# YulioTech/Yulio-Raytracer

Hardware: AMD Instinct MI355X
Metric: Mrays/s (Sponza stand-in 2048^2 64spp, closest+shadow queries) (higher is better)
Workload: dtype f32

## Files before the change

yulio-raytracer_amd/csrc/kernels/k_firsthit.h:

```cpp
#pragma once

#include "yrt_camera.h"
#include "yrt_shade.h"
#include "yrt_surface.h"
#include "yrt_traverse.h"

namespace yrt {

__global__ __launch_bounds__(64) void k_debug(SceneView sv, FrameView fv, int maxDepth, int spp,
                                             float* __restrict__ fbFloat, uint8_t* __restrict__ fbRGB8,
                                             int rgb8Stride) {
  const GpuRenderParams& rp = *fv.rp;
  const GpuCamera& cam = *fv.cam;
  const int tile = blockIdx.x * blockDim.x + threadIdx.x;
  if (tile >= rp.numTilesX * rp.numTilesY) return;
  DevRandom rnd;
  rnd.setSeed(tile * 1024);
  const int x0 = (tile % rp.numTilesX) * 16, y0 = (tile / rp.numTilesX) * 16;
  for (int dy = 0; dy < 16; dy++) {
    const int iy = y0 + dy;
    const float fy = iy * rp.rcpHeight;
    if (iy >= rp.height) continue;
    for (int dx = 0; dx < 16; dx++) {
      const int ix = x0 + dx;
      const float fx = ix * rp.rcpWidth;
      if (ix >= rp.width) continue;
      for (int i = 0; i < spp; i++) {
        V3 org, dir;
        camera_ray(cam, fx, fy, org, dir);
        float tnear = 0.f, tfar = __int_as_float(0x7f800000);
        Hit h;
        h.tri = -1;
        int id0 = -1, id1 = -1;
        for (int depth = 0; depth < maxDepth; depth++) {
          h = closest_hit(sv.qnodes, sv.tris, org, dir, tnear, tfar);
          if (h.tri < 0) {
            id0 = id1 = -1;
            break;
          }
          const int g = sv.triGeom[h.tri];
          id0 = g;
          id1 = h.tri - sv.geoms[g].triBase;
          if (depth + 1 < maxDepth) {
            const int4 idx = sv.indices[h.tri];
            const V3 p0 = ld3(sv.positions[idx.x]), p1 = ld3(sv.positions[idx.y]), p2 = ld3(sv.positions[idx.z]);
            V3 e1, e2;
            yrt_tri_edges(&p0.x, &p1.x, &p2.x, &e1.x, &e2.x);
            V3 Nf = normalize(cross(e1, e2));
            if (dot(-dir, Nf) < 0) Nf = -Nf;
            const float u1 = rnd.getFloat();
            const float u2 = rnd.getFloat();
            float pdf;
            const V3 norg = org + 0.999f * h.t * dir;
            dir = cosine_hemi(u1, u2, Nf, pdf);
            org = norg;
            tnear = 4.0f * kUlp;
            tfar = __int_as_float(0x7f800000);
          }
        }
        V3 c;
        if (id0 < 0) c = v3s(1.0f);
        else
          c = v3(((3434553u * ((unsigned)(id0 + id1 + 3243))) % 255) / 255.0f,
                 ((7342453u * ((unsigned)(id0 + id1 + 8237))) % 255) / 255.0f,
                 ((9234454u * ((unsigned)(id0 + id1 + 2343))) % 255) / 255.0f);
        if (fbFloat) {
          float* o = fbFloat + ((size_t)iy * rp.width + ix) * 3;
          o[0] = c.x;
          o[1] = c.y;
          o[2] = c.z;
        }
        if (fbRGB8) {
          uint8_t* o = fbRGB8 + (size_t)iy * rgb8Stride + 3 * ix;
          o[0] = (uint8_t)clampf(c.x * 255.0f, 0.0f, 255.0f);
          o[1] = (uint8_t)clampf(c.y * 255.0f, 0.0f, 255.0f);
          o[2] = (uint8_t)clampf(c.z * 255.0f, 0.0f, 255.0f);
        }
      }
    }
  }
}

__global__ __launch_bounds__(YRT_TRACE_BLOCK) void k_pick(SceneView sv, const GpuCamera* camp, float x, float y,
                                                          float4* out) {
  if (threadIdx.x != 0) return;
  V3 org, dir;
  camera_ray(*camp, x, y, org, dir);
  const Hit h = closest_hit(sv.qnodes, sv.tris, org, dir, 0.f, __int_as_float(0x7f800000));
  const V3 p = org + h.t * dir;
  out[0] = make_float4(p.x, p.y, p.z, __int_as_float(h.tri));
}

template <bool ALBEDO>
__global__ __launch_bounds__(YRT_TRACE_BLOCK) void k_guides(SceneView sv, const GpuCamera* camp, int width, int height,
                                                            float4* __restrict__ pos4, float4* __restrict__ nrm4,
                                                            float4* __restrict__ albedo4) {
  const long long i = (long long)blockIdx.x * blockDim.x + threadIdx.x;
  if (i >= (long long)width * height) return;
  const int y = (int)(i / width), x = (int)(i - (long long)y * width);
  V3 org, dir;
  camera_ray(*camp, (float(x) + 0.5f) / float(width), (float(y) + 0.5f) / float(height), org, dir);
  const Hit h = closest_hit(sv.qnodes, sv.tris, org, dir, 0.f, __int_as_float(0x7f800000));
  if (h.tri < 0) {
    pos4[i] = make_float4(0.f, 0.f, 0.f, __int_as_float(0x7f800000));
    nrm4[i] = make_float4(0.f, 0.f, 0.f, 0.f);
    if constexpr (ALBEDO) albedo4[i] = make_float4(0.f, 0.f, 0.f, 0.f);
    return;
  }
  DG dg;
  const float4* tsr = (const float4*)(sv.triShade + h.tri);
  const float4 r0 = tsr[0];
  const int g = __float_as_int(r0.w);
  post_intersect(sv, sv.geoms[g], tsr, r0, org, dir, h.t, h.u, h.v, h.tri, dg, false, 0.f);
  V3 n = dg.Ns;
  if (dot(n, dir) > 0.f) n = -n;
  pos4[i] = make_float4(dg.P.x, dg.P.y, dg.P.z, h.t);
  nrm4[i] = make_float4(n.x, n.y, n.z, 1.f);
  if constexpr (ALBEDO) {
    V3 a = v3s(0.f);
    if (dg.light < 0 && dg.material >= 0) {
      DG sdg = dg;
      if (dot(sdg.Ng, dir) > 0.f) {
        sdg.Ng = -sdg.Ng;
        sdg.Ns = -sdg.Ns;
      }
      BRDFSet bs;
      const GpuGeomRec& gr = sv.geomRecs[g];
      shade_material<YRT_ALL_MATS>(sv, gr.m, gr.t0, sdg.material, 0, sdg, bs);
#pragma unroll
      for (int k = 0; k < YRT_MAX_COMPS; ++k)
        if (k < bs.n && comp_type(bs.c[k].kind) == BT_DIFFUSE_REFLECTION) a = a + bs.c[k].R;
    }
    if (a == v3s(0.f)) a = v3s(1.f);
    albedo4[i] = make_float4(a.x, a.y, a.z, 1.f);
  }
}

}
```

yulio-raytracer_amd/csrc/kernels/k_shade.h:

```cpp
#pragma once

#include "yrt_camera.h"
#include "yrt_surface.h"

namespace yrt {

#ifndef YRT_SHADE_WAVES
#define YRT_SHADE_WAVES 4
#endif
#ifndef YRT_SHADE_WAVES_ALL
#define YRT_SHADE_WAVES_ALL 2
#endif
#ifndef YRT_SHADE_WAVES_MP
#define YRT_SHADE_WAVES_MP YRT_SHADE_WAVES
#endif
#ifdef YRT_PATH_DEBUG
__device__ int g_dbgPath[2] = {-1, -1};
__device__ float g_dbgTrace[32 * 32];
#endif

template <unsigned MM>
__global__ __launch_bounds__(YRT_BLOCK) __attribute__((amdgpu_waves_per_eu(
    MM == (YRT_ALL_MATS | YRT_ALL_LIGHTS) ? YRT_SHADE_WAVES_ALL
    : (MM & mat_bit(MAT_METALLIC_PAINT)) ? YRT_SHADE_WAVES_MP
                                         : YRT_SHADE_WAVES))) void k_shade(SceneView sv, FrameView fv, PathBuffers pb, BatchInfo bi,
                                                   int depthLevel) {
#ifdef YRT_SHADE_PROF
  unsigned long long sprof[8] = {0, 0, 0, 0, 0, 0, 0, 0};
  unsigned long long tprev = __builtin_amdgcn_s_memtime();
#define SPROF_AT(k)                                            \
  do {                                                         \
    const unsigned long long t_ = __builtin_amdgcn_s_memtime(); \
    sprof[k] += t_ - tprev;                                    \
    tprev = t_;                                                \
  } while (0)
#endif
#if defined(YRT_SHADE_PROF) && YRT_SHADE_PROF == 1
#define SPROF_MARK(k) SPROF_AT(k)
#else
#define SPROF_MARK(k) ((void)0)
#endif
#if defined(YRT_SHADE_PROF) && YRT_SHADE_PROF == 2
#define SPROF_FINE(k) SPROF_AT(k)
#else
#define SPROF_FINE(k) ((void)0)
#endif
  const YRT_CONST GpuRenderParams& rp = const_ref(fv.rp);
  __shared__ QMap qm;
  __shared__ float sstash[7 * YRT_MAX_COMPS * YRT_BLOCK];
  qmap_load(qm, pb.counters + qcounter_index(depthLevel, 0, 0), YRT_QSEGS);
  const int n = (int)qm.pre[YRT_QSEGS];
  const int cur = depthLevel & 1;
  const int numDirect = sv.numDirectLights;
  for (int base = blockIdx.x * blockDim.x; base < n; base += gridDim.x * blockDim.x) {
    const unsigned ql = (unsigned)base + threadIdx.x;
    const bool active = (int)ql < n;
    const int q = active ? qmap_phys(qm, pb.segCap, ql) : 0;
    const int oseg = qseg_of((unsigned)base + (threadIdx.x & ~63u));
    unsigned* nextCount = pb.counters + qcounter_index(depthLevel + 1, 0, oseg);
    unsigned* shadowCount = pb.counters + qcounter_index(depthLevel, 1, oseg);
    int path = 0;
    V3 org = v3s(0.f), dir = v3s(0.f), thr = v3s(0.f), L = v3s(0.f);
    int meta = 0, depth = 0, rec = 0, pixelId = 0, s = 0, medium = 0;
    bool ignoreVL = false, unbent = false, isHit = false, useDirect = false;
    bool haveL = false;
    float4 h = make_float4(0.f, 0.f, 0.f, 0.f);
    DG dg;
    BRDFSet bs;
    bs.n = 0;
#pragma unroll
    for (int k = 0; k < YRT_MAX_COMPS; ++k) {
      bs.c[k].kind = 0;
      bs.c[k].R = v3s(0.f);
      bs.c[k].a = bs.c[k].b = bs.c[k].c = 0.f;
    }
    V3 wo = v3s(0.f);
    int px = 0, py = 0;
    SPROF_MARK(7);
    SPROF_FINE(7);
    if (active) {
      path = pb.qPath[cur][q];
      h = pb.hit[q];
      if (depthLevel == 0) {
        thr = v3s(1.f);
        meta = 1 << 9;
        L = v3s(0.f);
        haveL = true;
      } else {
        const float4 t4 = pb.qThr[cur][q];
        thr = v3(t4.x, t4.y, t4.z);
        meta = __float_as_int(t4.w);
      }
      depth = meta & 255;
      ignoreVL = (meta >> 8) & 1;
      unbent = (meta >> 9) & 1;
      medium = (meta >> 10) & 0xFFFF;
      s = fastdiv(path, bi.divPixels);
      const int i = path - s * bi.numPixels;
      batch_pixel(rp, bi, i, px, py);
      pixelId = py * rp.width + px;
      isHit = __float_as_int(h.w) >= 0;
    }
    if (active && (isHit || sv.numEnvDir > 0)) {
      const float4 d = pb.qDir[cur][q];
      dir = v3(d.x, d.y, d.z);
      wo = -dir;
    }
    SPROF_MARK(0);
    if (active && !isHit) {
      {
        const int x = px, y = py;
        if (fv.backplateTexels && unbent) {
          rec = fv.pixelSets[pixelId] * rp.spp + s;
          const float fx = (float(x) + samp(fv, 0, rec)) * rp.rcpWidth;
          const float fy = (float(y) + samp(fv, 1, rec)) * rp.rcpHeight;
          const GpuImage& bp = fv.backplate;
          const int bx = max(0, min((int)(fx * (float)bp.width), bp.width - 1));
          const int by = max(0, min((int)(fy * (float)bp.height), bp.height - 1));
          float c[4];
          texel(bp, fv.backplateTexels, bx, by, c);
          if (!haveL) { const float4 l4 = pb.pathL[path]; L = v3(l4.x, l4.y, l4.z); haveL = true; }
          L = L + thr * v3(c[0], c[1], c[2]);
        } else if (!ignoreVL) {
          for (int j = 0; j < sv.numEnvLights; ++j) {
            if (!haveL) { const float4 l4 = pb.pathL[path]; L = v3(l4.x, l4.y, l4.z); haveL = true; }
            L = L + thr * env_Le<lights_of<MM>()>(sv, const_ref(sv.lights + const_ref(sv.envLights + j)), wo);
          }
          if (sv.numEnvZero > 0 && !(fabsf(thr.x) <= 3.40282347e38f && fabsf(thr.y) <= 3.40282347e38f && fabsf(thr.z) <= 3.40282347e38f)) {
            if (!haveL) { const float4 l4 = pb.pathL[path]; L = v3(l4.x, l4.y, l4.z); haveL = true; }
            L = L + thr * v3s(0.f);
          }
        }
      }
    }
    SPROF_MARK(1);
    bool backfacing = false;
    int g = 0;
    if (active && isHit) {
      const int gid = __float_as_int(h.w);
      const float4* tsr = (const float4*)(sv.triShade + gid);
      const float4 r0 = tsr[0];
      const float4 o = pb.qOrg[cur][q];
      org = v3(o.x, o.y, o.z);
      rec = fv.pixelSets[pixelId] * rp.spp + s;
      g = __float_as_int(r0.w);
      const GpuGeomRec& gr = sv.geomRecs[g];
      const int mat = gr.g.material;
      const bool wantT = mat >= 0 && (((MM & mat_bit(MAT_OBJ)) && gr.m.type == MAT_OBJ && gr.m.tex[4] >= 0) ||
                                      ((MM & mat_bit(MAT_BRUSHED_METAL)) && gr.m.type == MAT_BRUSHED_METAL));
      post_intersect(sv, gr.g, tsr, r0, org, dir, h.x, h.y, h.z, gid, dg, wantT, pb.qTime[0] ? samp(fv, 4, rec) : 0.f);
      if (dot(dg.Ng, dir) > 0.f) {
        backfacing = true;
        dg.Ng = -dg.Ng;
        dg.Ns = -dg.Ns;
      }
    }
    SPROF_MARK(2);
    if (active && isHit) {
      if (dg.material >= 0) shade_material<MM>(sv, sv.geomRecs[g].m, sv.geomRecs[g].t0, dg.material, medium, dg, bs);
      if (!ignoreVL && dg.light >= 0 && !backfacing) {
        const GpuLight& al = sv.lights[dg.light];
        if (!haveL) { const float4 l4 = pb.pathL[path]; L = v3(l4.x, l4.y, l4.z); haveL = true; }
        L = L + thr * v3(al.L[0], al.L[1], al.L[2]);
      }
#pragma unroll
      for (int k = 0; k < YRT_MAX_COMPS; ++k)
        if (k < bs.n) useDirect |= (comp_type(bs.c[k].kind) & BT_DIFFUSE) != 0;
      dg_frame(dg);
    }
    SPROF_MARK(3);

    bool cont = false;
    V3 nwi = v3s(0.f), nthr = v3s(0.f);
    int nmeta = 0;
    bool doSample = false;
    float4 sd = make_float4(0.f, 0.f, 0.f, 0.f);
    float sy = 0.f, ss = 0.f;
    if (active && isHit) {
      bool stop = depth >= rp.maxDepth - 1;
      if (!stop && rp.rrDepth > 0 && depth >= rp.rrDepth - 1) {
        const float qrr = fminf(reduce_max(thr) * 1.f * 1.f, .95f);
        if (samp(fv, 5 + rp.firstScatterTypeSampleID + depth, rec) >= qrr) stop = true;
      }
      if (!stop) {
        const int d2 = rp.firstScatterSampleID + depth;
        sd = samp_dir(fv, d2, rec);
        if constexpr ((comps_of(MM) & kCompsRawSy) != 0u) sy = samp(fv, 5 + rp.dim1D + 2 * d2 + 1, rec);
        ss = samp(fv, 5 + rp.firstScatterTypeSampleID + depth, rec);
        doSample = true;
      }
    }
    SPROF_FINE(0);
    float spdf = 0.f;
    uint32_t stype = 0;
    V3 sc = v3s(0.f);
    if (doSample)
      sc = set_sample<comps_of(MM)>(bs, sv.materials, wo, dg, sd, sy, ss, nwi, spdf, stype, sstash + threadIdx.x);
    SPROF_FINE(1);
    if (doSample) {
      {
        V3 c = sc;
        const float pdf = spdf;
        const uint32_t type = stype;
        if (!(c == v3s(0.f) || pdf <= 0.f)) {
          if (MM & mat_bit(MAT_DIELECTRIC)) {
            const float4 T = sv.media[medium];
            if (!(T.x == 1.f && T.y == 1.f && T.z == 1.f)) c = c * v3(yrt_powf(T.x, h.x), yrt_powf(T.y, h.x), yrt_powf(T.z, h.x));
            if ((type & BT_TRANSMISSION) && dg.material >= 0) {
              const GpuMaterial& mt = sv.materials[dg.material];
              if (mt.type == MAT_DIELECTRIC) medium = medium == mt.media[1] ? mt.media[0] : mt.media[1];
            }
          }
          nthr = thr * c * rcpf_(pdf);
          const bool nIgnore = (type & BT_DIFFUSE) != 0;
          const bool nUnbent = unbent && (nwi == dir);
          if (!(reduce_max(nthr) < rp.minContribution)) {
            cont = true;
            nmeta = (depth + 1) | ((nIgnore ? 1 : 0) << 8) | ((nUnbent ? 1 : 0) << 9) | (medium << 10);
          }
        }
      }
    }
    SPROF_MARK(4);
    if (haveL) pb.pathL[path] = make_float4(L.x, L.y, L.z, 0.f);
    auto cont_store = [&](unsigned nq) {
      if (pb.qTime[0]) pb.qTime[cur ^ 1][nq] = samp(fv, 4, rec);
      pb.qPath[cur ^ 1][nq] = path;
      pb.qOrg[cur ^ 1][nq] = make_float4(dg.P.x, dg.P.y, dg.P.z, dg.error * rp.epsilon);
      pb.qDir[cur ^ 1][nq] = make_float4(nwi.x, nwi.y, nwi.z, __int_as_float(0x7f800000));
      pb.qThr[cur ^ 1][nq] = make_float4(nthr.x, nthr.y, nthr.z, __int_as_float(nmeta));
    };
    auto light_term = [&](int k, V3& wi, float& tfar, V3& contrib) -> bool {
      const int li = const_ref(sv.directLights + k);
      const YRT_CONST GpuLight& lt = const_ref(sv.lights + li);
      const bool lit = active && isHit && useDirect && (lt.illumMask & dg.illumMask) != 0;
      V3 Ls = v3s(0.f);
      float pdf = 0.f;
      if (lit) {
        if (lt.precomputed >= 0) {
          const float* ls = fv.lightSamples + ((size_t)rec * fv.numLightSlots + lt.precomputed) * 8;
          wi = v3(ls[0], ls[1], ls[2]);
          pdf = ls[3];
          Ls = v3(ls[4], ls[5], ls[6]);
        } else {
          float4 lsd = make_float4(0.f, 0.f, 0.f, 0.f);
          float lsx = 0.f, lsy = 0.f;
          if ((1u << lt.type) & kLightsDir) lsd = samp_dir(fv, rp.lightSampleID, rec);
          if ((lights_of<MM>() & kLightsRawS) != 0u && ((1u << lt.type) & kLightsRawS)) {
            lsx = samp(fv, 5 + rp.dim1D + 2 * rp.lightSampleID, rec);
            lsy = samp(fv, 5 + rp.dim1D + 2 * rp.lightSampleID + 1, rec);
          }
          Ls = light_sample<lights_of<MM>()>(lt, dg, lsd, lsx, lsy, wi, pdf);
        }
      }
      SPROF_FINE(3);
      const bool lsOk = lit && !(Ls == v3s(0.f) || pdf == 0.f);
      V3 brdf = v3s(0.f);
      if (lsOk) brdf = set_eval<comps_of(MM)>(bs, sv.materials, wo, dg, wi, BT_DIFFUSE);
      SPROF_FINE(4);
      if (lsOk && !(brdf == v3s(0.f))) {
        const float r01 = hash_u01(rp.frameSeed, (uint32_t)pixelId, (uint32_t)s, (uint32_t)(depth * 64 + li));
        const float shadowRayJitterLength = 2.f * rp.tMaxShadowRay * rp.tMaxShadowJitter * r01 -
                                            rp.tMaxShadowRay * rp.tMaxShadowJitter;
        float tMax = rp.tMaxShadowRay + shadowRayJitterLength;
        const float dotProduct = dot(wi, ld3(rp.up));
        if (dotProduct <= 0.f) tMax += rp.tMaxShadowRay * 100.f * smoothstepf(0.f, 1.f, fabsf(dotProduct));
        tfar = tMax - dg.error * rp.epsilon;
        contrib = thr * Ls * brdf * rcpf_(pdf);
        return true;
      }
      return false;
    };
    auto shadow_store = [&](unsigned si, const V3& wi, float tfar, const V3& contrib) {
      if (pb.sTime) pb.sTime[si] = samp(fv, 4, rec);
      pb.sOrg[si] = make_float4(dg.P.x, dg.P.y, dg.P.z, dg.error * rp.epsilon);
      pb.sDir[si] = make_float4(wi.x, wi.y, wi.z, tfar);
      pb.sContrib[si] = make_float4(contrib.x, contrib.y, contrib.z, __int_as_float(path));
    };
    {
      bool got;
      const unsigned nq = oseg * pb.segCap + wave_append(nextCount, cont, got);
      if (got) cont_store(nq);
      SPROF_MARK(5);
      SPROF_FINE(2);
      for (int k = 0; k < numDirect; ++k) {
        V3 wi = v3s(0.f), contrib = v3s(0.f);
        float tfar = 0.f;
        const bool pred = light_term(k, wi, tfar, contrib);
        SPROF_FINE(5);
        bool sgot;
        const unsigned si = oseg * pb.shSegCap + wave_append(shadowCount, pred, sgot);
        if (sgot) shadow_store(si, wi, tfar, contrib);
        if (active && !pb.fuseShadow) pb.shFirst[(size_t)q * numDirect + k] = sgot ? (int)si : -1;
        SPROF_FINE(6);
      }
    }
    SPROF_MARK(6);
#ifdef YRT_PATH_DEBUG
    if (active && pixelId == g_dbgPath[0] && s == g_dbgPath[1] && depth < 32) {
      float* o = g_dbgTrace + depth * 32;
      if (!haveL) { const float4 l4 = pb.pathL[path]; L = v3(l4.x, l4.y, l4.z); }
      const float r[32] = {1.f, isHit ? (float)__float_as_int(h.w) : -1.f, h.x, h.y, h.z, thr.x, thr.y, thr.z,
                           dg.P.x, dg.P.y, dg.P.z, dg.Ns.x, dg.Ns.y, dg.Ns.z, L.x, L.y, L.z, nwi.x, nwi.y, nwi.z,
                           spdf, sc.x, sc.y, sc.z, nthr.x, nthr.y, nthr.z, dir.x, dir.y, dir.z, org.x, (float)useDirect};
      for (int k = 0; k < 32; ++k) o[k] = r[k];
    }
#endif
  }
#ifdef YRT_SHADE_PROF
  if (threadIdx.x == 0)
    for (int k = 0; k < 8; ++k) atomicAdd(&g_traceProfile[k], sprof[k]);
#endif
}

__global__ __launch_bounds__(YRT_BLOCK) void k_shadow_resolve(PathBuffers pb, int depthLevel, int numLights) {
  __shared__ QMap qm;
  qmap_load(qm, pb.counters + qcounter_index(depthLevel, 0, 0), YRT_QSEGS);
  const int n = (int)qm.pre[YRT_QSEGS];
  const int cur = depthLevel & 1;
  for (int ql = blockIdx.x * blockDim.x + threadIdx.x; ql < n; ql += gridDim.x * blockDim.x) {
    const int q = qmap_phys(qm, pb.segCap, (unsigned)ql);
    bool any = false;
    for (int li = 0; li < numLights; ++li) any |= pb.shFirst[(size_t)q * numLights + li] >= 0;
    if (!any) continue;
    float4* Lp = &pb.pathL[pb.qPath[cur][q]];
    const float4 l4 = *Lp;
    V3 L = v3(l4.x, l4.y, l4.z);
    for (int li = 0; li < numLights; ++li) {
      const int si = pb.shFirst[(size_t)q * numLights + li];
      if (si < 0 || pb.sOcc[si]) continue;
      const float4 c = pb.sContrib[si];
      L = L + v3(c.x, c.y, c.z);
    }
    *Lp = make_float4(L.x, L.y, L.z, 0.f);
  }
}

__device__ int g_dbgPixel[3] = {-1, -1, 0};
__device__ float4* g_dbgOut = nullptr;

__global__ __launch_bounds__(YRT_BLOCK) void k_resolve_pixels(FrameView fv, PathBuffers pb, BatchInfo bi,
                                                            float* __restrict__ fbFloat, uint8_t* __restrict__ fbRGB8,
                                                            int rgb8Stride, float4* __restrict__ accu, int accumulate) {
  const YRT_CONST GpuRenderParams& rp = const_ref(fv.rp);
  const size_t frameStride = (size_t)rp.width * rp.height;
  for (int i = blockIdx.x * blockDim.x + threadIdx.x; i < bi.numPixels; i += gridDim.x * blockDim.x) {
    int x, y, f;
    if (!batch_pixel(rp, bi, i, x, y, f)) continue;
    V3 L = v3s(0.f);
    for (int s = 0; s < rp.spp; ++s) {
      const float4 l4 = pb.pathL[(size_t)s * bi.numPixels + i];
      L = L + v3(l4.x, l4.y, l4.z);
    }
    if (g_dbgPixel[0] == y * rp.width + x && g_dbgPixel[1] == f && g_dbgOut)
      for (int s = 0; s < min(rp.spp, g_dbgPixel[2]); ++s) g_dbgOut[s] = pb.pathL[(size_t)s * bi.numPixels + i];
    const size_t pix = (size_t)f * frameStride + (size_t)y * rp.width + x;
    float4 a = make_float4(L.x, L.y, L.z, (float)rp.spp);
    if (accumulate) {
      const float4 c = accu[pix];
      a = make_float4(c.x + L.x, c.y + L.y, c.z + L.z, c.w + (float)rp.spp);
    }
    accu[pix] = a;
    V3 L0 = accumulate ? v3(a.x, a.y, a.z) * rcpf_(a.w) : L * rcpf_((float)rp.spp);
    if (rp.gamma != 1.0f) L0 = v3(yrt_powf(L0.x, rp.rcpGamma), yrt_powf(L0.y, rp.rcpGamma), yrt_powf(L0.z, rp.rcpGamma));
    if (rp.vignetting) {
      const float rw = rcpf_(0.5f * float(rp.width));
      const float vx = (float(x) - 0.5f * float(rp.width)) * rw, vy = (float(y) - 0.5f * float(rp.height)) * rw;
      const float d = sqrtf(vx * vx + vy * vy);
      L0 = L0 * yrt_powf(yrt_cosf(d * 0.5f), 3.0f);
    }
    if (fbFloat) {
      float* o = fbFloat + pix * 3;
      o[0] = L0.x;
      o[1] = L0.y;
      o[2] = L0.z;
    }
    if (fbRGB8) {
      uint8_t* o = fbRGB8 + ((size_t)f * rp.height + y) * rgb8Stride + 3 * x;
      o[0] = (uint8_t)clampf(L0.x * 255.0f, 0.0f, 255.0f);
      o[1] = (uint8_t)clampf(L0.y * 255.0f, 0.0f, 255.0f);
      o[2] = (uint8_t)clampf(L0.z * 255.0f, 0.0f, 255.0f);
    }
  }
}

#undef SPROF_AT
#undef SPROF_MARK
#undef SPROF_FINE

}
```

yulio-raytracer_amd/csrc/kernels/yrt_surface.h:

```cpp
#pragma once

#include "yrt_shade.h"
#include "yrt_wave.h"
#include "../common/yrt_tri_record.h"

namespace yrt {


struct TriRecordSource {
  static constexpr bool kTangentArrays = false;
  const float4* __restrict__ rec;
  float4 r0;
  __device__ __forceinline__ void edges(V3& e1, V3& e2, V3& dPdu, V3& dPdv) const {
    const float4 r1 = rec[1];
    e1 = v3(r0.x, r0.y, r0.z); e2 = v3(r1.x, r1.y, r1.z);
    dPdu = -e1; dPdv = e2;
  }
  __device__ __forceinline__ void normals(V3& n0, V3& n1, V3& n2) const {
    const float4 r2 = rec[2], r3 = rec[3], r4 = rec[4];
    n0 = v3(r2.x, r2.y, r2.z); n1 = v3(r2.w, r3.x, r3.y); n2 = v3(r3.z, r3.w, r4.x);
  }
  __device__ __forceinline__ void texcoords(float2& st0, float2& st1, float2& st2) const {
    const float4 r4 = rec[4], r5 = rec[5];
    st0 = make_float2(r4.y, r4.z); st1 = make_float2(r4.w, r5.x); st2 = make_float2(r5.y, r5.z);
  }
};

struct TriIndexedSource {
  static constexpr bool kTangentArrays = true;
  const SceneView& sv;
  const int4 idx;
  const float time;
  const bool moving;
  __device__ __forceinline__ void edges(V3& e1, V3& e2, V3& dPdu, V3& dPdv) const {
    V3 p0 = ld3(sv.positions[idx.x]), p1 = ld3(sv.positions[idx.y]), p2 = ld3(sv.positions[idx.z]);
    if (moving) {
      p0 = p0 + time * ld3(sv.motions[idx.x]);
      p1 = p1 + time * ld3(sv.motions[idx.y]);
      p2 = p2 + time * ld3(sv.motions[idx.z]);
    }
    yrt_tri_edges(&p0.x, &p1.x, &p2.x, &e1.x, &e2.x);
    dPdu = p1 - p0; dPdv = p2 - p0;
  }
  __device__ __forceinline__ void normals(V3& n0, V3& n1, V3& n2) const {
    n0 = ld3(sv.normals[idx.x]); n1 = ld3(sv.normals[idx.y]); n2 = ld3(sv.normals[idx.z]);
  }
  __device__ __forceinline__ void texcoords(float2& st0, float2& st1, float2& st2) const {
    st0 = sv.texcoords[idx.x]; st1 = sv.texcoords[idx.y]; st2 = sv.texcoords[idx.z];
  }
  __device__ __forceinline__ V3 tangent(int k, float w, float u, float v) const {
    return w * ld3(sv.tangents[2 * idx.x + k]) + u * ld3(sv.tangents[2 * idx.y + k]) +
           v * ld3(sv.tangents[2 * idx.z + k]);
  }
};

__device__ __forceinline__ void post_intersect(const SceneView& sv, const GpuGeom& geom,
                                               const float4* __restrict__ rec, float4 r0, V3 org, V3 dir, float t,
                                               float u, float v, int gid, DG& dg, bool wantTangents, float time) {
  dg.material = geom.material;
  dg.light = geom.light;
  dg.illumMask = geom.illumMask;
  dg.shadowMask = geom.shadowMask;
  dg.P = org + t * dir;
  dg.s = u; dg.t = v;
  dg.Tx = dg.Ty = v3s(0.f);
  auto mesh = [&](const auto src) {
    V3 e1, e2, dPdu, dPdv;
    src.edges(e1, e2, dPdu, dPdv);
    const float w = 1.0f - u - v;
    dg.Ns = dg.Ng = normalize(cross(e1, e2));
    const bool meshNormals = geom.kind == GEOM_MESH_NORMALS;
    if (meshNormals || (geom.flags & GF_NORMALS)) {
      V3 n0, n1, n2;
      src.normals(n0, n1, n2);
      V3 Ns = w * n0 + u * n1 + v * n2;
      const float len2 = dot(Ns, Ns);
      Ns = len2 > 0 ? Ns * rsqrtf_(len2) : dg.Ng;
      if (dot(Ns, dg.Ng) < 0) Ns = -Ns;
      dg.Ns = Ns;
    }
    if (meshNormals) {
      dg.Tx = dPdu; dg.Ty = dPdv;
      return;
    }
    float dsdu = 1, dtdu = 0, dsdv = 0, dtdv = 1;
    if (geom.flags & GF_TEXCOORDS) {
      float2 st0, st1, st2;
      src.texcoords(st0, st1, st2);
      dg.s = st0.x * w + st1.x * u + st2.x * v;
      dg.t = st0.y * w + st1.y * u + st2.y * v;
      dsdu = st1.x - st0.x; dtdu = st1.y - st0.y;
      dsdv = st2.x - st0.x; dtdv = st2.y - st0.y;
    }
    if (!wantTangents) return;
    const V3 dPds = normalize(dPdu * dtdv - dPdv * dtdu);
    dg.Tx = normalize(dPds - dot(dPds, dg.Ns) * dg.Ns);
    const V3 dPdt = normalize(dPdv * dsdu - dPdu * dsdv);
    dg.Ty = normalize(dPdt - dot(dPdt, dg.Ns) * dg.Ns);
    if constexpr (src.kTangentArrays) {
      if (geom.flags & GF_TANGENT_X) dg.Tx = src.tangent(0, w, u, v);
      if (geom.flags & GF_TANGENT_Y) dg.Ty = src.tangent(1, w, u, v);
    }
  };
  if (geom.kind == GEOM_TRIANGLE)
    dg.Ns = dg.Ng = v3(geom.Ng[0], geom.Ng[1], geom.Ng[2]);
  else if (geom.flags & (GF_MOTION | GF_TANGENT_X | GF_TANGENT_Y))
    mesh(TriIndexedSource{sv, sv.indices[gid], time, (geom.flags & GF_MOTION) != 0});
  else
    mesh(TriRecordSource{rec, r0});
  dg.error = fmaxf(fabsf(t), reduce_max(absv(dg.P)));
}

__device__ __forceinline__ void add_comp(BRDFSet& bs, int kind, uint32_t type, V3 R, float a = 0.f, float b = 0.f,
                                         float c = 0.f) {
  (void)type;
#pragma unroll
  for (int i = 0; i < YRT_MAX_COMPS; ++i) {
    const bool w = i == bs.n;
    bs.c[i].kind = w ? kind : bs.c[i].kind;
    bs.c[i].R = v3(w ? R.x : bs.c[i].R.x, w ? R.y : bs.c[i].R.y, w ? R.z : bs.c[i].R.z);
    bs.c[i].a = w ? a : bs.c[i].a;
    bs.c[i].b = w ? b : bs.c[i].b;
    bs.c[i].c = w ? c : bs.c[i].c;
  }
  bs.n = bs.n < YRT_MAX_COMPS ? bs.n + 1 : bs.n;
}

template <unsigned MM>
__device__ __forceinline__ void shade_material(const SceneView& sv, const GpuMaterial& m, const GpuTexture& t0, int matId,
                                               int medium, DG& dg, BRDFSet& bs) {
  bs.n = 0;
  const float idBits = __int_as_float(matId);
  switch (m.type) {
    case MAT_PLASTIC:
      if constexpr (!(MM & mat_bit(MAT_PLASTIC))) break;
      add_comp(bs, C_DIEL_LAYER_LAMB, BT_DIFFUSE_REFLECTION, v3(m.p[0], m.p[1], m.p[2]), m.p[6], m.p[7]);
      if (m.p[4] == 0.0f) add_comp(bs, C_DIEL_REFL, BT_SPECULAR_REFLECTION, v3s(0.f), m.p[8], 1.0f);
      else add_comp(bs, C_MICROFACET, BT_GLOSSY_REFLECTION, v3s(1.f), 1.0f, m.p[3], m.p[5]);
      break;
    case MAT_DIELECTRIC:
      if constexpr (!(MM & mat_bit(MAT_DIELECTRIC))) break;
      if (medium == m.media[0]) {
        add_comp(bs, C_DIEL_REFL, BT_SPECULAR_REFLECTION, v3s(0.f), m.p[8], 1.0f);
        add_comp(bs, C_DIEL_TRANS, BT_SPECULAR_TRANSMISSION, v3s(0.f), m.p[8]);
      } else {
        add_comp(bs, C_DIEL_REFL, BT_SPECULAR_REFLECTION, v3s(0.f), m.p[9], 1.0f);
        add_comp(bs, C_DIEL_TRANS, BT_SPECULAR_TRANSMISSION, v3s(0.f), m.p[9]);
      }
      break;
    case MAT_MIRROR:
      if constexpr (!(MM & mat_bit(MAT_MIRROR))) break;
      add_comp(bs, C_REFLECTION, BT_SPECULAR_REFLECTION, v3(m.p[0], m.p[1], m.p[2]));
      break;
    case MAT_METAL:
      if constexpr (!(MM & mat_bit(MAT_METAL))) break;
      if (m.p[9] == 0.0f) add_comp(bs, C_CONDUCTOR, BT_SPECULAR_REFLECTION, v3(m.p[0], m.p[1], m.p[2]), 0.f, 0.f, idBits);
      else add_comp(bs, C_MICRO_COND, BT_GLOSSY_REFLECTION, v3(m.p[0], m.p[1], m.p[2]), m.p[10], 0.f, idBits);
      break;
    case MAT_BRUSHED_METAL:
      if constexpr (!(MM & mat_bit(MAT_BRUSHED_METAL))) break;
      if (m.p[9] == 0.0f || m.p[10] == 0.0f)
        add_comp(bs, C_CONDUCTOR, BT_SPECULAR_REFLECTION, v3(m.p[0], m.p[1], m.p[2]), 0.f, 0.f, idBits);
      else
        add_comp(bs, C_MICRO_ANISO, BT_GLOSSY_REFLECTION, v3(m.p[0], m.p[1], m.p[2]), m.p[11], m.p[12], idBits);
      break;
    case MAT_VELVET:
      if constexpr (!(MM & mat_bit(MAT_VELVET))) break;
      add_comp(bs, C_MINNAERT, BT_DIFFUSE_REFLECTION, v3(m.p[0], m.p[1], m.p[2]), m.p[3]);
      add_comp(bs, C_VELVETY, BT_DIFFUSE_REFLECTION, v3(m.p[4], m.p[5], m.p[6]), m.p[7]);
      break;
    case MAT_MATTE:
      if constexpr (!(MM & mat_bit(MAT_MATTE))) break;
      add_comp(bs, C_LAMBERT, BT_DIFFUSE_REFLECTION, v3(m.p[0], m.p[1], m.p[2]));
      break;
    case MAT_MATTE_TEXTURED:
      if constexpr (!(MM & mat_bit(MAT_MATTE_TEXTURED))) break;
      if (m.tex[0] >= 0) {
        float c[4];
        tex_get_rec(t0, sv.texels, sv.texQuads, m.p[2] * dg.s + m.p[0], m.p[3] * dg.t + m.p[1], c);
        add_comp(bs, C_LAMBERT, BT_DIFFUSE_REFLECTION, v3(c[0], c[1], c[2]));
      }
      break;
    case MAT_METALLIC_PAINT:
      if constexpr (!(MM & mat_bit(MAT_METALLIC_PAINT))) break;
      add_comp(bs, C_DIEL_REFL, BT_SPECULAR_REFLECTION, v3s(0.f), m.p[4], 1.0f);
      add_comp(bs, C_DIEL_LAYER_LAMB, BT_DIFFUSE_REFLECTION, v3(m.p[0], m.p[1], m.p[2]), m.p[5], m.p[6]);
      break;
    case MAT_METALLIC_GLITTER:
      if constexpr (!(MM & mat_bit(MAT_METALLIC_GLITTER))) break;
      add_comp(bs, C_DIEL_REFL, BT_SPECULAR_REFLECTION, v3s(0.f), m.p[4], 1.0f);
      add_comp(bs, C_DIEL_LAYER_LAMB, BT_DIFFUSE_REFLECTION, v3(m.p[0], m.p[1], m.p[2]), m.p[5], m.p[6]);
      add_comp(bs, C_DIEL_LAYER_GLITTER, BT_GLOSSY_REFLECTION, v3(m.p[7], m.p[8], m.p[9]), m.p[5], m.p[6], m.p[10]);
      break;
    case MAT_OBJ: {
      if constexpr (!(MM & mat_bit(MAT_OBJ))) break;
      float c[4];
      if (m.tex[4] >= 0) {
        tex_get(sv.textures, sv.images, sv.texels, sv.texQuads, m.tex[4], dg.s, dg.t, c);
        const V3 b = v3(2.0f * c[0] - 1.0f, 2.0f * c[1] - 1.0f, 2.0f * c[2] - 1.0f);
        dg.Ns = normalize(b.x * dg.Tx + b.y * dg.Ty + b.z * dg.Ns);
      }
      float d = m.p[0];
      if (m.tex[0] >= 0) {
        tex_get_rec(t0, sv.texels, sv.texQuads, dg.s, dg.t, c);
        d *= c[0];
      }
      if (d < 1.0f) add_comp(bs, C_TRANSMISSION, BT_SPECULAR_TRANSMISSION, v3s(1.0f - d));
      V3 Kd = d * v3(m.p[1], m.p[2], m.p[3]);
      if (m.tex[1] >= 0) {
        tex_get(sv.textures, sv.images, sv.texels, sv.texQuads, m.tex[1], dg.s, dg.t, c);
        Kd = Kd * v3(c[0], c[1], c[2]);
      }
      if (Kd != v3s(0.f)) add_comp(bs, C_LAMBERT, BT_DIFFUSE_REFLECTION, Kd);
      float Ns = m.p[7];
      if (m.tex[3] >= 0) {
        tex_get(sv.textures, sv.images, sv.texels, sv.texQuads, m.tex[3], dg.s, dg.t, c);
        Ns *= c[0];
      }
      V3 Ks = d * v3(m.p[4], m.p[5], m.p[6]);
      if (m.tex[2] >= 0) {
        tex_get(sv.textures, sv.images, sv.texels, sv.texQuads, m.tex[2], dg.s, dg.t, c);
        Ks = Ks * v3(c[0], c[1], c[2]);
      }
      if (Ks != v3s(0.f)) add_comp(bs, C_SPECULAR, BT_GLOSSY_REFLECTION, Ks, Ns);
      break;
    }
    case MAT_UBER: {
      if constexpr (!(MM & mat_bit(MAT_UBER))) break;
      float dc[4] = {m.p[0], m.p[1], m.p[2], 1.f};
      float alpha = 1.f, opacity = 0.f;
      if (m.tex[0] >= 0) {
        tex_get_rec(t0, sv.texels, sv.texQuads, m.p[5] * dg.s + m.p[3], m.p[6] * dg.t + m.p[4], dc);
        alpha = dc[3];
        opacity = 1.f - alpha;
      }
      add_comp(bs, C_LAMBERT, BT_DIFFUSE_REFLECTION, v3(dc[0] * alpha, dc[1] * alpha, dc[2] * alpha));
      if (alpha < 1.f) add_comp(bs, C_CONST_DIEL_TRANS, BT_SPECULAR_TRANSMISSION, v3s(opacity));
      if (m.p[9] > 0.f) add_comp(bs, C_DIEL_REFL, BT_SPECULAR_REFLECTION, v3s(0.f), m.p[11], alpha * m.p[9]);
      else if (m.p[8] == 0.f) add_comp(bs, C_DIEL_REFL, BT_SPECULAR_REFLECTION, v3s(0.f), m.p[11], alpha);
      else add_comp(bs, C_MICROFACET, BT_GLOSSY_REFLECTION, v3s(alpha), 1.f, m.p[7], m.p[10]);
      break;
    }
    case MAT_THIN_DIELECTRIC: {
      if constexpr (!(MM & mat_bit(MAT_THIN_DIELECTRIC))) break;
      add_comp(bs, C_DIEL_REFL, BT_SPECULAR_REFLECTION, v3s(0.f), m.p[10], 1.0f);
      float dc[4] = {m.p[0], m.p[1], m.p[2], 1.f};
      if (m.tex[0] >= 0)
        tex_get_rec(t0, sv.texels, sv.texQuads, m.p[5] * dg.s + m.p[3], m.p[6] * dg.t + m.p[4], dc);
      const float tr = m.p[9];
      const V3 T = v3(dc[0] * tr, dc[1] * tr, dc[2] * tr);
      add_comp(bs, C_THIN_DIEL_TRANS, BT_SPECULAR_TRANSMISSION, v3(yrt_logf(T.x), yrt_logf(T.y), yrt_logf(T.z)), m.p[10],
               m.p[8]);
      break;
    }
    default:
      break;
  }
}

__device__ __forceinline__ void img_get(const SceneView& sv, int image, int x, int y, float c[4]) {
  texel(sv.images[image], sv.texels, x, y, c);
}

template <class LT>
__device__ __forceinline__ V3 hdri_Le(const SceneView& sv, const LT& lt, V3 wo) {
  const A3 w2l = ldA3(lt.w2l);
  const V3 wi = xfmVector(w2l, -wo);
  const float theta = yrt_acosf(clampf(wi.y, -1.0f, 1.0f));
  float phi = yrt_atan2f(-wi.z, -wi.x);
  if (phi < 0) phi += 2.0f * kPi;
  const float u = 1.0f - (phi * kOneOverTwoPi);
  const float v = theta * kOneOverPi;
  const int width = lt.hdriW, height = lt.hdriH;
  int x = max(0, min((int)(u * width), width - 1));
  int xNext = x + 1;
  if (xNext == width) xNext = 0;
  const float alpha = u * width - x;
  int y = max(0, min((int)(v * height), height - 1));
  int yNext = y + 1;
  if (yNext == height) yNext = height - 1;
  const float beta = v * height - y;
  float c0[4], c1[4], c2[4], c3[4];
  img_get(sv, lt.image, x, y, c0);
  img_get(sv, lt.image, xNext, y, c1);
  img_get(sv, lt.image, xNext, yNext, c2);
  img_get(sv, lt.image, x, yNext, c3);
  V3 r;
  float* rr = &r.x;
#pragma unroll
  for (int k = 0; k < 3; ++k) {
    const float temp0 = beta * c3[k] + (1 - beta) * c0[k];
    const float temp1 = beta * c2[k] + (1 - beta) * c1[k];
    rr[k] = lt.L[k] * (alpha * temp1 + (1 - alpha) * temp0);
  }
  return r;
}

constexpr unsigned kAllLights = 0x7Fu;
template <unsigned MM>
constexpr unsigned lights_of() { return (MM >> 16) & kAllLights; }
template <unsigned LM, class LT>
__device__ __forceinline__ V3 env_Le(const SceneView& sv, const LT& lt, V3 wo) {
  if ((LM & (1u << LIGHT_AMBIENT)) && lt.type == LIGHT_AMBIENT) return v3(lt.L[0], lt.L[1], lt.L[2]);
  if ((LM & (1u << LIGHT_DISTANT)) && lt.type == LIGHT_DISTANT)
    return dot(-wo, ld3(lt.e1)) >= lt.bsphere[1] ? v3(lt.L[0], lt.L[1], lt.L[2]) : v3s(0.f);
  if ((LM & (1u << LIGHT_HDRI)) && lt.type == LIGHT_HDRI) return hdri_Le(sv, lt, wo);
  return v3s(0.f);
}

constexpr unsigned kLightsRawS = (1u << LIGHT_TRIANGLE) | (1u << LIGHT_DISTANT);
constexpr unsigned kLightsDir = (1u << LIGHT_AMBIENT) | (1u << LIGHT_DISTANT);
template <unsigned LM, class LT>
__device__ __forceinline__ V3 light_sample(const LT& lt, const DG& dg, float4 sd, float sx, float sy, V3& wi,
                                           float& pdf) {
  if ((LM & (1u << LIGHT_AMBIENT)) && lt.type == LIGHT_AMBIENT) {
    wi = cosine_hemi_dg(sd, dg, pdf);
    return v3(lt.L[0], lt.L[1], lt.L[2]);
  }
  if ((LM & (1u << LIGHT_TRIANGLE)) && lt.type == LIGHT_TRIANGLE) {
    const V3 A = ld3(lt.v0), B = ld3(lt.v1), C = ld3(lt.v2);
    const float su = sqrtf(sx);
    const V3 d = (C + (1.0f - su) * (A - C) + (sy * su) * (B - C)) - dg.P;
    const float tMax = length(d);
    const float dDotNg = dot(d, ld3(lt.Ng));
    if (dDotNg >= 0) {
      pdf = 0.f;
      wi = v3s(0.f);
      return v3s(0.f);
    }
    wi = d * rcpf_(tMax);
    pdf = 2.0f * tMax * tMax * tMax * rcpf_(fabsf(dDotNg));
    return v3(lt.L[0], lt.L[1], lt.L[2]);
  }
  if ((LM & (1u << LIGHT_POINT)) && lt.type == LIGHT_POINT) {
    const V3 d = ld3(lt.v0) - dg.P;
    const float distance = length(d);
    wi = d / distance;
    pdf = distance * distance;
    return v3(lt.L[0], lt.L[1], lt.L[2]);
  }
  if ((LM & (1u << LIGHT_SPOT)) && lt.type == LIGHT_SPOT) {
    const V3 d = ld3(lt.v0) - dg.P;
    const float distance = length(d);
    wi = d * rcpf_(distance);
    pdf = distance * distance;
    const float cosAngle = dot(wi, ld3(lt.e1));
    const float cosMin = lt.bsphere[0], cosMax = lt.bsphere[1];
    if (cosMin != cosMax) return v3(lt.L[0], lt.L[1], lt.L[2]) * clampf((cosAngle - cosMax) * rcpf_(cosMin - cosMax));
    if (cosAngle > cosMin) return v3(lt.L[0], lt.L[1], lt.L[2]);
    return v3s(0.f);
  }
  if ((LM & (1u << LIGHT_DIRECTIONAL)) && lt.type == LIGHT_DIRECTIONAL) {
    wi = ld3(lt.e1);
    pdf = 1.0f;
    return v3(lt.L[0], lt.L[1], lt.L[2]);
  }
  if ((LM & (1u << LIGHT_DISTANT)) && lt.type == LIGHT_DISTANT) {
    const float angle = lt.bsphere[0];
    const float cosTheta = 1.0f - sy * (1.0f - yrt_cosf(angle));
    const float sinTheta = cos2sin(cosTheta);
    const V3 l = v3(sd.x * sinTheta, sd.y * sinTheta, cosTheta);
    pdf = rcpf_(4.0f * kPi * sqrf(yrt_sinf(0.5f * angle)));
    wi = mul(frame(ld3(lt.e1)), l);
    return v3(lt.L[0], lt.L[1], lt.L[2]);
  }
  pdf = 0.f;
  wi = v3s(0.f);
  return v3s(0.f);
}

}
```

yulio-raytracer_amd/csrc/kernels/yrt_wave.h:

```cpp
#pragma once

#include <hip/hip_runtime.h>

#include "yrt_kernels.h"

namespace yrt {

#ifndef YRT_BLOCK
#define YRT_BLOCK 64
#endif

__device__ __forceinline__ int lane_id() { return __lane_id(); }
__device__ __forceinline__ float opaque_zero() {
  float z;
  asm volatile("v_mov_b32 %0, 0" : "=v"(z));
  return z;
}
__device__ __forceinline__ unsigned lanes_below(unsigned long long m) {
  return __builtin_amdgcn_mbcnt_hi((unsigned)(m >> 32), __builtin_amdgcn_mbcnt_lo((unsigned)m, 0u));
}

__device__ __forceinline__ unsigned long long ballot(bool p) { return __builtin_amdgcn_ballot_w64(p); }

__device__ __forceinline__ unsigned wave_append(unsigned* counter, bool pred, bool& got) {
  const unsigned long long mask = ballot(pred);
  got = pred;
  if (mask == 0) return 0;
  const int lane = lane_id();
  const int leader = __ffsll((long long)mask) - 1;
  unsigned base = 0;
  if (lane == leader) base = atomicAdd(counter, (unsigned)__popcll(mask));
  base = __shfl(base, leader, 64);
  return base + (unsigned)__popcll(mask & ((1ull << lane) - 1ull));
}

struct QMap {
  unsigned pre[YRT_QSEGS + 1];
};

__device__ __forceinline__ void qmap_load(QMap& m, const unsigned* counts, int numSegs) {
  if (threadIdx.x == 0) {
    unsigned c[YRT_QSEGS];
#pragma unroll
    for (int k = 0; k < YRT_QSEGS; ++k) c[k] = k < numSegs ? counts[(size_t)k * YRT_QCSTRIDE] : 0u;
    unsigned acc = 0;
#pragma unroll
    for (int k = 0; k < YRT_QSEGS; ++k) {
      m.pre[k] = acc;
      acc += c[k];
    }
    m.pre[YRT_QSEGS] = acc;
  }
  __syncthreads();
}

__device__ __forceinline__ int qmap_phys(const QMap& m, int segCap, unsigned q) {
  int lo = 0;
#pragma unroll
  for (int step = YRT_QSEGS / 2; step > 0; step >>= 1)
    if (m.pre[lo + step] <= q) lo += step;
  return lo * segCap + (int)(q - m.pre[lo]);
}

__device__ __forceinline__ int qseg_of(unsigned q) { return (int)((q >> 6) % YRT_QSEGS); }

struct DevRandom {
  int seed, state;
  int table[32];
  __device__ void setSeed(int s) {
    const int a = 16807, m = 2147483647, q = 127773, r = 2836;
    if (s == 0) seed = 1;
    else if (s < 0) seed = -s;
    else seed = s;
    for (int j = 32 + 7; j >= 0; j--) {
      int k = seed / q;
      seed = a * (seed - k * q) - r * k;
      if (seed < 0) seed += m;
      if (j < 32) table[j] = seed;
    }
    state = table[0];
  }
  __device__ int getInt() {
    const int a = 16807, m = 2147483647, q = 127773, r = 2836;
    int k = seed / q;
    seed = a * (seed - k * q) - r * k;
    if (seed < 0) seed += m;
    int j = state / (1 + (2147483647 - 1) / 32);
    state = table[j];
    table[j] = seed;
    return state;
  }
  __device__ int getInt(int limit) { return getInt() % limit; }
  __device__ float getFloat() { return fminf(getInt() / 2147483647.0f, 1.0f - kUlp); }
};

__device__ __forceinline__ uint32_t mix32(uint32_t h) {
  h ^= h >> 16; h *= 0x7feb352dU; h ^= h >> 15; h *= 0x846ca68bU; h ^= h >> 16;
  return h;
}
__device__ __forceinline__ float hash_u01(uint32_t seed, uint32_t pixel, uint32_t sample, uint32_t depthLight) {
  uint32_t h = mix32(seed ^ 0x9e3779b9U);
  h = mix32(h ^ pixel);
  h = mix32(h ^ (sample * 0x85ebca6bU));
  h = mix32(h ^ (depthLight * 0xc2b2ae35U));
  return (float)(h >> 8) * (1.0f / 16777216.0f);
}

#define YRT_CONST __attribute__((address_space(4)))
template <class T>
__device__ __forceinline__ const YRT_CONST T& const_ref(const T* p) {
  return *(const YRT_CONST T*)p;
}

template <class F>
__device__ __forceinline__ V3 ld3(const F* p) { return v3(p[0], p[1], p[2]); }
__device__ __forceinline__ V3 ld3(const float4& p) { return v3(p.x, p.y, p.z); }
template <class F>
__device__ __forceinline__ A3 ldA3(const F* m) {
  return a3(l3(v3(m[0], m[1], m[2]), v3(m[3], m[4], m[5]), v3(m[6], m[7], m[8])), v3(m[9], m[10], m[11]));
}

#if defined(YRT_PROFILE) && defined(YRT_SHADE_PROF)
#error "YRT_PROFILE and YRT_SHADE_PROF share the profile counters: build one at a time"
#endif
#if defined(YRT_PROFILE) || defined(YRT_SHADE_PROF)
__device__ unsigned long long g_traceProfile[8];
#endif

}
```

Measured before the change: 7694.

## Burst-load triangle and geometry records in shade, merge queue appends, defer pathL store

The shade kernel now loads the full six-float4 triangle shading record up front and pulls only the geometry/material/texture pieces it needs as int4 bursts. Each piece set is chosen per material mask, replacing scattered field loads. The continuation and first shadow append are combined into one ballot/leader/shuffle sequence, and the pathL store moves to the end for non-metallic-paint variants. This aims to cut memory latency stalls and atomic round trips, at the cost of more registers and possibly lower occupancy.

```diff
diff --git a/yulio-raytracer_amd/csrc/kernels/k_firsthit.h b/yulio-raytracer_amd/csrc/kernels/k_firsthit.h
--- a/yulio-raytracer_amd/csrc/kernels/k_firsthit.h
+++ b/yulio-raytracer_amd/csrc/kernels/k_firsthit.h
@@ -111,7 +111,7 @@
   const float4* tsr = (const float4*)(sv.triShade + h.tri);
   const float4 r0 = tsr[0];
   const int g = __float_as_int(r0.w);
-  post_intersect(sv, sv.geoms[g], tsr, r0, org, dir, h.t, h.u, h.v, h.tri, dg, false, 0.f);
+  post_intersect(sv, sv.geoms[g], TriRecordLazySource{tsr, r0}, org, dir, h.t, h.u, h.v, h.tri, dg, false, 0.f);
   V3 n = dg.Ns;
   if (dot(n, dir) > 0.f) n = -n;
   pos4[i] = make_float4(dg.P.x, dg.P.y, dg.P.z, h.t);
diff --git a/yulio-raytracer_amd/csrc/kernels/k_shade.h b/yulio-raytracer_amd/csrc/kernels/k_shade.h
--- a/yulio-raytracer_amd/csrc/kernels/k_shade.h
+++ b/yulio-raytracer_amd/csrc/kernels/k_shade.h
@@ -14,6 +14,22 @@
 #ifndef YRT_SHADE_WAVES_MP
 #define YRT_SHADE_WAVES_MP YRT_SHADE_WAVES
 #endif
+#ifndef YRT_SHADE_BURST_REC
+#define YRT_SHADE_BURST_REC 1
+#endif
+#ifndef YRT_SHADE_BURST_GEOM
+#define YRT_SHADE_BURST_GEOM 1
+#endif
+#ifndef YRT_SHADE_STORES_LAST
+#define YRT_SHADE_STORES_LAST 1
+#endif
+template <unsigned MM>
+constexpr bool shade_burst_rec() { return YRT_SHADE_BURST_REC != 0; }
+template <unsigned MM>
+constexpr bool shade_burst_geom() { return YRT_SHADE_BURST_GEOM != 0; }
+template <unsigned MM>
+constexpr bool shade_stores_last() { return YRT_SHADE_STORES_LAST != 0 && !(MM & mat_bit(MAT_METALLIC_PAINT)); }
+
 #ifdef YRT_PATH_DEBUG
 __device__ int g_dbgPath[2] = {-1, -1};
 __device__ float g_dbgTrace[32 * 32];
@@ -136,19 +152,41 @@
     SPROF_MARK(1);
     bool backfacing = false;
     int g = 0;
+    GpuMaterial gm = {};
+    GpuTexture gt0 = {};
     if (active && isHit) {
       const int gid = __float_as_int(h.w);
       const float4* tsr = (const float4*)(sv.triShade + gid);
-      const float4 r0 = tsr[0];
+      TriRecordSource trs;
+      trs.r[0] = tsr[0];
+      if constexpr (shade_burst_rec<MM>()) {
+#pragma unroll
+        for (int k = 1; k < 6; ++k) trs.r[k] = tsr[k];
+      }
+      const float4 r0 = trs.r[0];
       const float4 o = pb.qOrg[cur][q];
       org = v3(o.x, o.y, o.z);
       rec = fv.pixelSets[pixelId] * rp.spp + s;
       g = __float_as_int(r0.w);
-      const GpuGeomRec& gr = sv.geomRecs[g];
-      const int mat = gr.g.material;
-      const bool wantT = mat >= 0 && (((MM & mat_bit(MAT_OBJ)) && gr.m.type == MAT_OBJ && gr.m.tex[4] >= 0) ||
-                                      ((MM & mat_bit(MAT_BRUSHED_METAL)) && gr.m.type == MAT_BRUSHED_METAL));
-      post_intersect(sv, gr.g, tsr, r0, org, dir, h.x, h.y, h.z, gid, dg, wantT, pb.qTime[0] ? samp(fv, 4, rec) : 0.f);
+      const float time = pb.qTime[0] ? samp(fv, 4, rec) : 0.f;
+      auto want_tangents = [&](int mat, const GpuMaterial& m) {
+        return mat >= 0 && (((MM & mat_bit(MAT_OBJ)) && m.type == MAT_OBJ && m.tex[4] >= 0) ||
+                            ((MM & mat_bit(MAT_BRUSHED_METAL)) && m.type == MAT_BRUSHED_METAL));
+      };
+      auto post = [&](const auto& geom, bool wantT) {
+        if constexpr (shade_burst_rec<MM>())
+          post_intersect(sv, geom, trs, org, dir, h.x, h.y, h.z, gid, dg, wantT, time);
+        else
+          post_intersect(sv, geom, TriRecordLazySource{tsr, r0}, org, dir, h.x, h.y, h.z, gid, dg, wantT, time);
+      };
+      if constexpr (shade_burst_geom<MM>()) {
+        GeomHead gh;
+        geom_burst<MM>(sv.geomRecs + g, gh, gm, gt0);
+        post(gh, want_tangents(gh.material, gm));
+      } else {
+        const GpuGeomRec& gr = sv.geomRecs[g];
+        post(gr.g, want_tangents(gr.g.material, gr.m));
+      }
       if (dot(dg.Ng, dir) > 0.f) {
         backfacing = true;
         dg.Ng = -dg.Ng;
@@ -157,7 +195,10 @@
     }
     SPROF_MARK(2);
     if (active && isHit) {
-      if (dg.material >= 0) shade_material<MM>(sv, sv.geomRecs[g].m, sv.geomRecs[g].t0, dg.material, medium, dg, bs);
+      if (dg.material >= 0) {
+        if constexpr (shade_burst_geom<MM>()) shade_material<MM>(sv, gm, gt0, dg.material, medium, dg, bs);
+        else shade_material<MM>(sv, sv.geomRecs[g].m, sv.geomRecs[g].t0, dg.material, medium, dg, bs);
+      }
       if (!ignoreVL && dg.light >= 0 && !backfacing) {
         const GpuLight& al = sv.lights[dg.light];
         if (!haveL) { const float4 l4 = pb.pathL[path]; L = v3(l4.x, l4.y, l4.z); haveL = true; }
@@ -222,7 +263,8 @@
       }
     }
     SPROF_MARK(4);
-    if (haveL) pb.pathL[path] = make_float4(L.x, L.y, L.z, 0.f);
+    if constexpr (!shade_stores_last<MM>())
+      if (haveL) pb.pathL[path] = make_float4(L.x, L.y, L.z, 0.f);
     auto cont_store = [&](unsigned nq) {
       if (pb.qTime[0]) pb.qTime[cur ^ 1][nq] = samp(fv, 4, rec);
       pb.qPath[cur ^ 1][nq] = path;
@@ -277,7 +319,37 @@
       pb.sDir[si] = make_float4(wi.x, wi.y, wi.z, tfar);
       pb.sContrib[si] = make_float4(contrib.x, contrib.y, contrib.z, __int_as_float(path));
     };
-    {
+    auto shadow_append = [&](int k, bool pred, const V3& wi, float tfar, const V3& contrib) {
+      bool sgot;
+      const unsigned si = oseg * pb.shSegCap + wave_append(shadowCount, pred, sgot);
+      if (sgot) shadow_store(si, wi, tfar, contrib);
+      if (active && !pb.fuseShadow) pb.shFirst[(size_t)q * numDirect + k] = sgot ? (int)si : -1;
+    };
+    if constexpr (shade_stores_last<MM>()) {
+      V3 wi = v3s(0.f), contrib = v3s(0.f);
+      float tfar = 0.f;
+      const bool pred = numDirect > 0 && light_term(0, wi, tfar, contrib);
+      SPROF_FINE(5);
+      unsigned nq, si;
+      wave_append2(nextCount, cont, nq, shadowCount, pred, si);
+      nq += oseg * pb.segCap;
+      si += oseg * pb.shSegCap;
+      if (cont) cont_store(nq);
+      SPROF_MARK(5);
+      SPROF_FINE(2);
+      if (numDirect > 0) {
+        if (pred) shadow_store(si, wi, tfar, contrib);
+        if (active && !pb.fuseShadow) pb.shFirst[(size_t)q * numDirect] = pred ? (int)si : -1;
+      }
+      SPROF_FINE(6);
+      for (int k = 1; k < numDirect; ++k) {
+        const bool predk = light_term(k, wi, tfar, contrib);
+        SPROF_FINE(5);
+        shadow_append(k, predk, wi, tfar, contrib);
+        SPROF_FINE(6);
+      }
+      if (haveL) pb.pathL[path] = make_float4(L.x, L.y, L.z, 0.f);
+    } else {
       bool got;
       const unsigned nq = oseg * pb.segCap + wave_append(nextCount, cont, got);
       if (got) cont_store(nq);
@@ -288,10 +360,7 @@
         float tfar = 0.f;
         const bool pred = light_term(k, wi, tfar, contrib);
         SPROF_FINE(5);
-        bool sgot;
-        const unsigned si = oseg * pb.shSegCap + wave_append(shadowCount, pred, sgot);
-        if (sgot) shadow_store(si, wi, tfar, contrib);
-        if (active && !pb.fuseShadow) pb.shFirst[(size_t)q * numDirect + k] = sgot ? (int)si : -1;
+        shadow_append(k, pred, wi, tfar, contrib);
         SPROF_FINE(6);
       }
     }
diff --git a/yulio-raytracer_amd/csrc/kernels/yrt_surface.h b/yulio-raytracer_amd/csrc/kernels/yrt_surface.h
--- a/yulio-raytracer_amd/csrc/kernels/yrt_surface.h
+++ b/yulio-raytracer_amd/csrc/kernels/yrt_surface.h
@@ -8,6 +8,21 @@
 
 
 struct TriRecordSource {
+  static constexpr bool kTangentArrays = false;
+  float4 r[6];
+  __device__ __forceinline__ void edges(V3& e1, V3& e2, V3& dPdu, V3& dPdv) const {
+    e1 = v3(r[0].x, r[0].y, r[0].z); e2 = v3(r[1].x, r[1].y, r[1].z);
+    dPdu = -e1; dPdv = e2;
+  }
+  __device__ __forceinline__ void normals(V3& n0, V3& n1, V3& n2) const {
+    n0 = v3(r[2].x, r[2].y, r[2].z); n1 = v3(r[2].w, r[3].x, r[3].y); n2 = v3(r[3].z, r[3].w, r[4].x);
+  }
+  __device__ __forceinline__ void texcoords(float2& st0, float2& st1, float2& st2) const {
+    st0 = make_float2(r[4].y, r[4].z); st1 = make_float2(r[4].w, r[5].x); st2 = make_float2(r[5].y, r[5].z);
+  }
+};
+
+struct TriRecordLazySource {
   static constexpr bool kTangentArrays = false;
   const float4* __restrict__ rec;
   float4 r0;
@@ -54,9 +69,15 @@
   }
 };
 
-__device__ __forceinline__ void post_intersect(const SceneView& sv, const GpuGeom& geom,
-                                               const float4* __restrict__ rec, float4 r0, V3 org, V3 dir, float t,
-                                               float u, float v, int gid, DG& dg, bool wantTangents, float time) {
+struct GeomHead {
+  int32_t kind, material, light, flags, illumMask, shadowMask;
+  const float* Ng;
+};
+
+template <class GEOM, class REC>
+__device__ __forceinline__ void post_intersect(const SceneView& sv, const GEOM& geom, const REC& rec, V3 org, V3 dir,
+                                               float t, float u, float v, int gid, DG& dg, bool wantTangents,
+                                               float time) {
   dg.material = geom.material;
   dg.light = geom.light;
   dg.illumMask = geom.illumMask;
@@ -107,8 +128,52 @@
   else if (geom.flags & (GF_MOTION | GF_TANGENT_X | GF_TANGENT_Y))
     mesh(TriIndexedSource{sv, sv.indices[gid], time, (geom.flags & GF_MOTION) != 0});
   else
-    mesh(TriRecordSource{rec, r0});
+    mesh(rec);
   dg.error = fmaxf(fabsf(t), reduce_max(absv(dg.P)));
+}
+
+template <unsigned MM>
+constexpr int mat_p_quads() {
+  int n = 0;
+  constexpr unsigned one = mat_bit(MAT_MATTE) | mat_bit(MAT_MIRROR) | mat_bit(MAT_MATTE_TEXTURED);
+  constexpr unsigned two = mat_bit(MAT_VELVET) | mat_bit(MAT_OBJ) | mat_bit(MAT_METALLIC_PAINT);
+  constexpr unsigned three = mat_bit(MAT_PLASTIC) | mat_bit(MAT_DIELECTRIC) | mat_bit(MAT_METAL) |
+                             mat_bit(MAT_METALLIC_GLITTER) | mat_bit(MAT_UBER) | mat_bit(MAT_THIN_DIELECTRIC);
+  constexpr unsigned four = mat_bit(MAT_BRUSHED_METAL);
+  if (MM & one) n = 1;
+  if (MM & two) n = 2;
+  if (MM & three) n = 3;
+  if (MM & four) n = 4;
+  return n;
+}
+constexpr unsigned kMatsQ4 = mat_bit(MAT_OBJ) | mat_bit(MAT_DIELECTRIC);
+constexpr unsigned kMatsT0 = mat_bit(MAT_MATTE_TEXTURED) | mat_bit(MAT_OBJ) | mat_bit(MAT_UBER) | mat_bit(MAT_THIN_DIELECTRIC);
+
+template <unsigned MM>
+__device__ __forceinline__ void geom_burst(const GpuGeomRec* __restrict__ gr, GeomHead& gh, GpuMaterial& m,
+                                           GpuTexture& t0) {
+  static_assert(sizeof(GpuGeom) == 48 && sizeof(GpuMaterial) == 128 && sizeof(GpuGeomRec) == 208, "piece offsets below");
+  const int4* __restrict__ q = (const int4*)gr;
+  constexpr int NP = mat_p_quads<MM>();
+  const int4 q0 = q[0], q1 = q[1], q3 = q[3];
+  int4 q4 = make_int4(0, 0, 0, 0), qt0 = q4, qt1 = q4;
+  float4 qp[4];
+  if constexpr ((MM & kMatsQ4) != 0u) q4 = q[4];
+#pragma unroll
+  for (int k = 0; k < 4; ++k) qp[k] = k < NP ? ((const float4*)gr)[5 + k] : make_float4(0.f, 0.f, 0.f, 0.f);
+  if constexpr ((MM & kMatsT0) != 0u) { qt0 = q[11]; qt1 = q[12]; }
+  gh.kind = q0.x; gh.material = q0.y; gh.light = q0.z; gh.flags = q0.w;
+  gh.illumMask = q1.z; gh.shadowMask = q1.w;
+  gh.Ng = gr->g.Ng;
+  m.type = q3.x; m.tex[0] = q3.y; m.tex[1] = q3.z; m.tex[2] = q3.w;
+  if constexpr ((MM & kMatsQ4) != 0u) { m.tex[3] = q4.x; m.tex[4] = q4.y; m.media[0] = q4.z; m.media[1] = q4.w; }
+#pragma unroll
+  for (int k = 0; k < NP; ++k) { m.p[4 * k] = qp[k].x; m.p[4 * k + 1] = qp[k].y; m.p[4 * k + 2] = qp[k].z; m.p[4 * k + 3] = qp[k].w; }
+  if constexpr ((MM & kMatsT0) != 0u) {
+    t0.image = qt0.x; t0.filter = qt0.y; t0.invert = qt0.z; t0.width = qt0.w;
+    t0.height = qt1.x; t0.format = qt1.y;
+    t0.offset = (int64_t)(((uint64_t)(uint32_t)qt1.w << 32) | (uint32_t)qt1.z);
+  }
 }
 
 __device__ __forceinline__ void add_comp(BRDFSet& bs, int kind, uint32_t type, V3 R, float a = 0.f, float b = 0.f,
diff --git a/yulio-raytracer_amd/csrc/kernels/yrt_wave.h b/yulio-raytracer_amd/csrc/kernels/yrt_wave.h
--- a/yulio-raytracer_amd/csrc/kernels/yrt_wave.h
+++ b/yulio-raytracer_amd/csrc/kernels/yrt_wave.h
@@ -32,6 +32,31 @@
   if (lane == leader) base = atomicAdd(counter, (unsigned)__popcll(mask));
   base = __shfl(base, leader, 64);
   return base + (unsigned)__popcll(mask & ((1ull << lane) - 1ull));
+}
+
+__device__ __forceinline__ void wave_append2(unsigned* counter0, bool pred0, unsigned& slot0, unsigned* counter1,
+                                             bool pred1, unsigned& slot1) {
+  const unsigned long long m0 = ballot(pred0), m1 = ballot(pred1);
+  slot0 = slot1 = 0;
+  if ((m0 | m1) == 0) return;
+  const int lane = lane_id();
+  const int leader = __ffsll((long long)(m0 | m1)) - 1;
+  unsigned b0 = 0, b1 = 0;
+  if (lane == leader) {
+    if (m0 != 0 && m1 != 0) {
+      b0 = atomicAdd(counter0, (unsigned)__popcll(m0));
+      b1 = atomicAdd(counter1, (unsigned)__popcll(m1));
+    } else if (m0 != 0) {
+      b0 = atomicAdd(counter0, (unsigned)__popcll(m0));
+    } else {
+      b1 = atomicAdd(counter1, (unsigned)__popcll(m1));
+    }
+  }
+  b0 = __shfl(b0, leader, 64);
+  b1 = __shfl(b1, leader, 64);
+  const unsigned long long below = (1ull << lane) - 1ull;
+  slot0 = b0 + (unsigned)__popcll(m0 & below);
+  slot1 = b1 + (unsigned)__popcll(m1 & below);
 }
 
 struct QMap {
```

Result: faster. 7998 (median of 6 runs) (+4.0%).
